# unixpickle/learn-nerf

Hardware: AMD Instinct MI355X
Metric: ray-samples/s (NeRF train step: fwd + bwd + Adam, 4096 rays x 192 samples per GPU) (higher is better)
Workload: dtype bf16; 1 GPU; vanilla NeRF coarse64+fine128 train step (BASELINE.json configs[1]); rays_per_gpu=4096, coarse_samples=64, fine_samples=128, global_batch_rays=4096, parallelism=dp1, precision=bf16 MFMA, fp32 accumulate/master weights

## Files before the change

### learn-nerf_amd/csrc/layout_host.cpp

```cpp
#include <stdint.h>
#include <string.h>

#include "dense_plan.h"
#include "fast_math.h"
#include "hashgrid_plan.h"
#include "nerf_wgrad.h"
#include "ngp_layout.h"

using namespace lnrf;

static WgradList wgrad_list_of(int which, int64_t n_tiles) {
  return which == 0 ? wgrad_list_split(n_tiles) : which == 1 ? wgrad_list_ls_finish(n_tiles)
       : which == 2 ? wgrad_list_ref_trunk(n_tiles) : which == 3 ? wgrad_list_ref_normal(n_tiles)
                                                                 : wgrad_list_ref_dir(n_tiles);
}
template <int NXF, int NYF, int WI, int WO>
static int64_t wgrad_count_owners(const WgradProblem& pb, int32_t* count, int64_t n) {
  int64_t outside = 0;
  int64_t i;
  auto hit = [&](bool owned) {
    if (!owned) return;
    if (i >= 0 && i < n) ++count[i];
    else ++outside;
  };
  for (int w = 0; w < kWaves; ++w)
    for (int j = 0; j < kWgradWaveTiles<NXF, NYF, WI, WO>; ++j) {
      const WgradTile tile = wgrad_tile<NXF, NYF, WI, WO>(w, j);
      if (!tile.real) continue;
      for (int lane = 0; lane < 64; ++lane) {
        const int colr = lane & 31, hh = lane >> 5;
        const WgradOwner<NerfWgradEpi, WgradProblem> own(pb, tile.ot, colr);
        if (tile.bias && pb.do_bias) hit(own.bias(hh, i));
        for (int qq = 0; qq < 16; ++qq) hit(own.weight(pb, tile.it, hh, qq, i));
      }
    }
  return outside;
}

template <int P>
static int64_t ngp_count_owners(const NgpWgradProblem& pb, int64_t dense_off, int32_t* count, int64_t n) {
  constexpr int NO = kNgpWgrad[P].nyf / 2, NT = ngp_wgrad_tiles(P);
  int64_t outside = 0;
  auto hit = [&](int part, int64_t i) {
    if (i >= 0 && i < n) ++count[part * n + i];
    else ++outside;
  };
  for (int w4 = 0; w4 < 4; ++w4)
    for (int lane = 0; lane < 64; ++lane) {
      const int colr = lane & 31, hh = lane >> 5;
      const int tile_id = w4 % NT, part = w4 / NT;
      const int it = tile_id / NO, ot = tile_id % NO;
      int out_idx = -1, out_dim = 1;
      int64_t w_off = 0, b_off = 0;
      NgpWgradEpi::cols(pb, ot, colr, out_idx, out_dim, w_off, b_off);
      w_off -= dense_off;
      b_off -= dense_off;
      if (it == 0 && hh == 0 && out_idx >= 0) hit(part, b_off + out_idx);
      for (int qq = 0; qq < 16; ++qq) {
        const int r = ngp_acc_row(qq, hh);
        const int f = 2 * it + (r >> 4);
        const int in_idx = NgpWgradEpi::row(pb, f, r & 15);
        if (out_idx >= 0 && in_idx >= 0) hit(part, w_off + (int64_t)in_idx * out_dim + out_idx);
      }
    }
  return outside;
}
static bool ngp_enc_dim_ok(int enc_dim) { return enc_dim >= 1 && enc_dim <= 32; }
// ... 19 lines not shown
                                                                                             : fwd_cons_base(s);
}
int lnrf_host_bwd_layer_info(int t, int what) {
  return what == 0 ? bwd_nk(t) : what == 1 ? bwd_no(t) : what == 2 ? bwd_base(t) : bwd_dense(t);
}
int lnrf_host_fwd_weight_index(int g, int lane, int j) { return fwd_stream_index(g, lane, j, false); }
int lnrf_host_bwd_weight_index(int g, int lane, int j) { return bwd_stream_index(g, lane, j, false); }
int lnrf_host_fwd_bias_index(int i) { return bias_block_index(i, false); }
int lnrf_host_nrm_frags(void) { return kNrmFrags; }
int lnrf_host_nrm_weight_index(int g, int lane, int j) { return nrm_stream_index(g, lane, j); }
int64_t lnrf_host_stream_indices(int stream, int ref, int32_t* out) {
  const int frags[8] = {kFwdFrags, kBwdFrags, kFwd3Frags, 0, kNrmFrags, kDirFwdFrags, kDirBwdFrags, 0};
  if (stream < 0 || stream > 7) return -1;
  if (stream == 3 || stream == 7) {
    const int n = stream == 3 ? kBiasFloats : kDirBiasFloats;
    for (int i = 0; out && i < n; ++i) out[i] = stream == 3 ? bias_block_index(i, ref != 0) : dir_bias_index(i);
    return n;
  }
  const int64_t n = (int64_t)frags[stream] * 512;
  for (int64_t e = 0; out && e < n; ++e) {
    const int g = (int)(e >> 9), lane = (int)((e >> 3) & 63), j = (int)(e & 7);
    out[e] = stream == 0 ? fwd_stream_index(g, lane, j, ref != 0) : stream == 1 ? bwd_stream_index(g, lane, j, ref != 0)
           : stream == 2 ? fwd3_stream_index(g, lane, j, ref != 0) : stream == 4 ? nrm_stream_index(g, lane, j)
           : stream == 5 ? dir_fwd_weight_index(g, lane, j) : dir_bwd_weight_index(g, lane, j);
  }
  return n;
}
int64_t lnrf_host_pack_offset(int what) {
  const int64_t v[17] = {kPackFwdOff, kPackBwdOff, kPackBiasOff, kPackBytes, kPack3BiasOff, kPack3Bytes,
                         kRefPackNrmOff, kRefPackDirFwdOff, kRefPackDirBwdOff, kRefPackDirBiasOff, kRefPackBytes,
                         kRef3FwdOff, kRef3BiasOff, kRef3NrmOff, kRef3DirOff, kRef3DirBiasOff, kRef3Bytes};
  return what >= 0 && what < 17 ? v[what] : -1;
}
int lnrf_host_xemb_feat(int ks, int h, int j) { return xemb_feat(ks, h, j); }
int lnrf_host_save_slot(int what, int arg) {
  return what == 0 ? kSaveXin : what == 1 ? kSaveH + 16 * arg : what == 2 ? kSaveZ : what == 3 ? kSaveDin
       : what == 4 ? kSaveH10 : what == 5 ? kSaveMask : kSaveSlots;
}
int lnrf_host_grad_slot(int what, int arg) {
  return what == 0 ? kGradDy11 : what == 1 ? kGradDy10m : what == 2 ? grad_dy_slot(arg) : kGradSlots;
}
int lnrf_host_dir_slot(int what) {
  const int v[7] = {kDirSaveXin, kDirSaveH, kDirSaveMask, kDirSaveSlots, kDirGradDy10, kDirGradDy9, kDirGradSlots};
  return what >= 0 && what < 7 ? v[what] : -1;
}
int lnrf_host_demb_feat(int ks, int h, int j) { return demb_feat(ks, h, j); }
int lnrf_host_hidden_feat(int ks, int h, int j) { return hidden_feat(ks, h, j); }
int lnrf_host_dump_info(int what) { return what == 0 ? kFragBytes : what == 1 ? kTileCols : kWaves; }
int lnrf_host_mask_bit(int ks, int j) { return 16 * (ks >> 1) + 8 * (ks & 1) + j; }
int lnrf_host_dump_lane_off(int slot, int c, int hh) { return dump_lane_off(slot, c, hh); }
void lnrf_host_sincos_pe(float r, float* s, float* c) { lnrf::sincos_pe(r, s, c); }

int lnrf_host_wgrad_const(int what) {
  const int v[8] = {kWgradMaxBlocks, kSlabMaxTiles, kSlabMaxTO, kParamCount, kDirW9, kDirB9, kDirW10, kDirB10};
  return v[what];
}
int lnrf_host_wgrad_list(int which, int64_t n_tiles, int32_t* out) {
  const WgradList list = wgrad_list_of(which, n_tiles);
  for (int i = 0; i < list.args.n_problems; ++i) {
    const WgradProblem& pb = list.args.p[i];
    int32_t* o = out + 6 * i;
    o[0] = pb.first_block; o[1] = pb.n_blocks; o[4] = pb.do_bias; o[5] = 0;
    switch (pb.shape) {
#define X(name, id, NXF, NYF, WI, WO, SPI) case name: o[2] = WgShape<name>::TI * WgShape<name>::TO; o[3] = WgShape<name>::TO; break;
      LNRF_WGRAD_SHAPES(X, X)
#undef X
      default: return -1;
    }
    switch (pb.shape) {
#define X(name) case name:
      LNRF_WGRAD_LS_SHAPES(X, X) o[5] = 1; break;
#undef X
      default: break;
    }
  }
  return list.args.n_problems;
}
int64_t lnrf_host_ngp_stream_indices(int stream, int enc_dim, int32_t* out) {
  if (stream < 0 || stream > 2 || !ngp_enc_dim_ok(enc_dim)) return -1;
  const NgpOffsets off = ngp_offsets(enc_dim, 0);
  const int ne = ngp_ne(enc_dim);
  const int64_t n = stream == 2 ? kNgpBiasFloats : (int64_t)kNgpStreamFrags * 512;
  for (int64_t e = 0; out && e < n; ++e) {
    const int g = (int)(e >> 9), lane = (int)((e >> 3) & 63), j = (int)(e & 7);
    out[e] = (int32_t)(stream == 0 ? ngp_fwd_stream_index(g, lane, j, off, enc_dim, ne)
                     : stream == 1 ? ngp_bwd_stream_index(g, lane, j, off, enc_dim, ne) : ngp_bias_index((int)e, off));
  }
  return n;
}
int64_t lnrf_host_ngp_pack_offset(int what) {
  const int64_t v[7] = {kNgpPackBiasOff, kNgpPackBytes, kNgpSplitBiasOff, kNgpSplitBytes, kNgpStreamFrags,
                        kNgpSplitMaxFrags / 2, kNgpMaxParts};
  return what >= 0 && what < 7 ? v[what] : -1;
}
int64_t lnrf_host_ngp_wgrad_owners(int enc_dim, int32_t* count, int64_t n) {
  if (!ngp_enc_dim_ok(enc_dim)) return -1;
  const int64_t dense_off = 1001;
  const NgpWgradArgs a = ngp_wgrad_args(ngp_offsets(enc_dim, dense_off), enc_dim);
  return ngp_count_owners<0>(a.p[0], dense_off, count, n) + ngp_count_owners<1>(a.p[1], dense_off, count, n) +
         ngp_count_owners<2>(a.p[2], dense_off, count, n) + ngp_count_owners<3>(a.p[3], dense_off, count, n) +
         ngp_count_owners<4>(a.p[4], dense_off, count, n);
}
int lnrf_host_ngp_parts_plan(int enc_dim, int32_t* out) {
  if (!ngp_enc_dim_ok(enc_dim)) return -1;
  const NgpPartsPlan pl = ngp_parts_plan(ngp_offsets(enc_dim, 1001), 1001);
  for (int i = 0; i < kNgpLayers; ++i) {
    int32_t* o = out + 4 * i;
// ... 86 lines not shown
```

### learn-nerf_amd/csrc/nerf_bwd_ls.hip

```cpp
#include "nerf_chain.h"

namespace lnrf {

constexpr int kLsWaves = 4;
constexpr int kLsThreads = kLsWaves * 64;
constexpr int kLsStages = 8;
constexpr int kLsLag = 2;
constexpr int kLsDist = kLsLag + 1;
constexpr int kLsBufs = kLsDist + 1;
constexpr int kLsTileBytes = 32 * kFragBytes;
constexpr int kLsPollOff = kLsBufs * kLsTileBytes;
constexpr int kLsLds = kLsPollOff + 5 * 256;
constexpr unsigned kLsMaxSpins = 1u << 18;
constexpr int kLsSlabWaveFloats = 16 * kSlabTileFloats + 2 * 64;
constexpr int64_t kLsSlabBlockBytes = (int64_t)kLsWaves * kLsSlabWaveFloats * (int64_t)sizeof(float);
constexpr int kLsCounterStride = 32;

struct LsJob {
  const char* packed;
  const char* save;
  char* gdump;
  unsigned* counters;
  float* slabs;
  unsigned* status;
// ... 350 lines not shown
  const int out = 32 * b + colr;
  if (bias) {
    bs += __shfl_xor(bs, 32, 64);
    if (hh == 0) grads[dense_b_off(l) + out] += bs;
  }
  const int it = 2 * w + a;
#pragma unroll
  for (int qq = 0; qq < 16; ++qq) {
    const int r = (qq & 3) + 8 * (qq >> 2) + 4 * hh;
    grads[dense_w_off(l) + (int64_t)(32 * it + r) * 256 + out] += acc[qq];
  }
}
__global__ __launch_bounds__(256) void nerf_ls_reduce_kernel(const float* __restrict__ slabs, int pipelines,
                                                             float* __restrict__ grads) {
  __shared__ float lds[3 * 17 * 64];
  ls_fold_block<4>(blockIdx.x, slabs, pipelines, grads, lds);
}

struct LsFoldArgs {
  WgradArgs w[2];
  const float* small_slabs[2];
  const float* ls_slabs[2];
  float* grads[2];
  int pipelines[2];
};
__global__ __launch_bounds__(64 * kSlabReduceWaves) void nerf_ls_fold_kernel(LsFoldArgs a) {
  __shared__ float lds[(kSlabReduceWaves - 1) * 17 * 64];
  const int k = blockIdx.y;
  const int n_small = a.w[k].n_problems * kWaves * kSlabMaxTiles;
  const int bid = blockIdx.x;
  if (bid < n_small) {
    const int prob = bid / (kWaves * kSlabMaxTiles), w = bid / kSlabMaxTiles % kWaves, j = bid % kSlabMaxTiles;
    const WgradProblem pb = a.w[k].p[prob];
    switch (pb.shape) {
#define X(name)                                                                                                    \
  case name:                                                                                                       \
    wgrad_reduce_tile<WgShape<name>::NXF, WgShape<name>::NYF, WgShape<name>::WI, WgShape<name>::WO, NerfWgradEpi>( \
        pb, w, j, a.small_slabs[k], a.grads[k], lds);                                                              \
    break;
      LNRF_WGRAD_LS_SHAPES(X, default: X)
#undef X
    }
  } else if (bid - n_small < kLsStages * 64) {
    ls_fold_block<kSlabReduceWaves>(bid - n_small, a.ls_slabs[k], a.pipelines[k], a.grads[k], lds);
  }
}

struct BwdHeadSeq {
  static constexpr int count = bwd_cons_base(2);
  static constexpr int at(int c) { return bwd_seq(c); }
};
constexpr int kBwdHeadStages = bwd_base(2) / kStageFrags;

__global__ __launch_bounds__(kThreads) void nerf_bwd_head_kernel(
    const char* __restrict__ packed, const char* __restrict__ save, const float* __restrict__ density,
    const float* __restrict__ rgb, const float* __restrict__ g_density, const float* __restrict__ g_rgb,
    int64_t M, int64_t n_tiles, char* __restrict__ gdump, unsigned* __restrict__ zero_words, int n_zero_words) {
  const int tid = threadIdx.x;
  const int lane = tid & 63;
  const int wave = __builtin_amdgcn_readfirstlane(tid >> 6);
  const int64_t tile = (int64_t)blockIdx.x * kWaves + wave;
  for (int i = blockIdx.x * kThreads + tid; i < n_zero_words; i += gridDim.x * kThreads) zero_words[i] = 0u;
  Ring<kBwdHeadStages, BwdHeadSeq> ring;
  ring.stream = packed + kPackBwdOff;
  ring.wave = wave;
  ring.lane = lane;
  const DumpAddr gd{gdump, n_tiles, tile, lane & 31, lane >> 5, kGradTileSlots};
  bwd_chain_tile<true>(ring, gd, save, n_tiles, density, rgb, g_density, g_rgb, M, tile, lane);
}

}

using namespace lnrf;

#ifdef LNRF_TIMELINE
extern "C" int lnrf_debug_set_ls_timeline(void* buf) {
  hipError_t e = hipMemcpyToSymbol(HIP_SYMBOL(lnrf::g_ls_timeline_buf), &buf, sizeof(buf));
  return e == hipSuccess ? LNRF_OK : hip_fail(e, "hipMemcpyToSymbol(g_ls_timeline_buf)");
}
#endif

constexpr int kLsMaxPipelines = 64;
static int ls_pipelines_for_device(int need, int* out) {
  int cus = 0;
  if (int rc = cu_count(&cus)) return rc;
  *out = cus / kLsStages < kLsMaxPipelines ? cus / kLsStages : kLsMaxPipelines;
  if (*out < need) {
    set_error("layer-stationary backward: the device has too few CUs for a pipeline of 8 per model");
    return LNRF_ERR_UNSUPPORTED;
  }
  return LNRF_OK;
}

constexpr int64_t kLsCounterWords = (int64_t)kLsMaxPipelines * kLsStages * kLsCounterStride;
constexpr int64_t kLsCounterBytes = (kLsCounterWords + 64) * (int64_t)sizeof(unsigned);
struct LsScratch {
  int64_t small_slabs, counters, status, ls_slabs, bytes;
};
static LsScratch ls_scratch(int64_t m) {
  LsScratch s;
  s.small_slabs = (int64_t)kGradSlots * padded_tiles(m) * kFragBytes;
  s.counters = s.small_slabs + kWgradSlabBytes;
  s.status = s.counters + kLsCounterWords * (int64_t)sizeof(unsigned);
  s.ls_slabs = s.counters + kLsCounterBytes;
  s.bytes = s.ls_slabs + (int64_t)kLsMaxPipelines * kLsStages * kLsSlabBlockBytes;
  return s;
}
static LsJob ls_job(const void* packed, const void* save, void* scratch, int64_t m, int pipelines) {
  const LsScratch at = ls_scratch(m);
  char* sc = (char*)scratch;
  return LsJob{(const char*)packed, (const char*)save, sc, reinterpret_cast<unsigned*>(sc + at.counters),
               reinterpret_cast<float*>(sc + at.ls_slabs), reinterpret_cast<unsigned*>(sc + at.status), padded_tiles(m),
               pipelines};
}

extern "C" int64_t lnrf_nerf_bwd_ls_scratch_bytes(const lnrf_nerf_shape* s, int64_t m) {
  return nerf_shape_fused(s) ? ls_scratch(m).bytes : -1;
}
extern "C" int64_t lnrf_nerf_bwd_ls_status_offset(const lnrf_nerf_shape* s, int64_t m) {
  return nerf_shape_fused(s) ? ls_scratch(m).status : -1;
}
int64_t lnrf::ls_scratch_bytes(int64_t m) { return ls_scratch(m).bytes; }
float* lnrf::ls_small_slabs(void* scratch, int64_t m) {
  return reinterpret_cast<float*>((char*)scratch + ls_scratch(m).small_slabs);
}

int lnrf::launch_ls_pipeline(const void* packed, const void* save, void* scratch, int64_t m, float* grads, hipStream_t st) {
  int total = 0;
  int rc = ls_pipelines_for_device(1, &total);
  if (!rc) rc = set_max_dynamic_lds(nerf_bwd_ls_kernel, kLsLds);
  if (rc) return rc;
  LsArgs a;
  a.n_jobs = 1;
  a.total_pipelines = total;
  a.job[0] = a.job[1] = ls_job(packed, save, scratch, m, total);
  hipError_t e = hipMemsetAsync(a.job[0].counters, 0, kLsCounterBytes, st);
  if (e != hipSuccess) return hip_fail(e, "hipMemsetAsync(counters)");
  hipLaunchKernelGGL(nerf_bwd_ls_kernel, dim3((unsigned)(total * kLsStages)), dim3(kLsThreads), kLsLds, st, a);
  LNRF_LAUNCH_CHECK();
  hipLaunchKernelGGL(nerf_ls_reduce_kernel, dim3(kLsStages * 64), dim3(256), 0, st, (const float*)a.job[0].slabs, total, grads);
  LNRF_LAUNCH_CHECK();
  return LNRF_OK;
}

namespace {
struct LsModel {
  const void* packed;
  const void* save;
  const float *density, *rgb, *g_density, *g_rgb;
  int64_t m;
  void* scratch;
  float* grads;
};
}

static int ls_backward(const LsModel* mdl, int n_models, int phases, hipStream_t st) {
  constexpr int kHeadLds = kRingBytes + round_up(kBiasFloats * 4, 1024);
  int total = 0;
  int rc = ls_pipelines_for_device(n_models, &total);
  if (!rc) rc = set_max_dynamic_lds(nerf_bwd_head_kernel, kHeadLds);
  if (!rc) rc = set_max_dynamic_lds(nerf_bwd_ls_kernel, kLsLds);
  if (rc) return rc;
  int pipes[2] = {total, 0};
  if (n_models == 2) {
    const double share = (double)mdl[0].m / (double)(mdl[0].m + mdl[1].m);
    pipes[0] = (int)(total * share + 0.5);
    if (pipes[0] < 1) pipes[0] = 1;
    if (pipes[0] > total - 1) pipes[0] = total - 1;
    pipes[1] = total - pipes[0];
  }
  LsArgs a;
  a.n_jobs = n_models;
  a.total_pipelines = total;
  for (int k = 0; k < n_models; ++k) {
    const LsModel& md = mdl[k];
    const LsJob& j = a.job[k] = ls_job(md.packed, md.save, md.scratch, md.m, pipes[k]);
    if (phases & 1) {
      hipLaunchKernelGGL(nerf_bwd_head_kernel, dim3((unsigned)(j.n_tiles / kWaves)), dim3(kThreads), kHeadLds, st, j.packed,
                         j.save, md.density, md.rgb, md.g_density, md.g_rgb, md.m, j.n_tiles, j.gdump, j.counters,
                         (phases & 2) ? (int)(kLsCounterBytes / sizeof(unsigned)) : 0);
      LNRF_LAUNCH_CHECK();
    }
    if ((phases & 3) == 2) {
      hipError_t e = hipMemsetAsync(j.counters, 0, kLsCounterBytes, st);
      if (e != hipSuccess) return hip_fail(e, "hipMemsetAsync(counters)");
    }
  }
  if (n_models == 1) a.job[1] = a.job[0];
  if (phases & 2) {
    hipLaunchKernelGGL(nerf_bwd_ls_kernel, dim3((unsigned)(total * kLsStages)), dim3(kLsThreads), kLsLds, st, a);
    LNRF_LAUNCH_CHECK();
  }
  if (!(phases & 4)) return LNRF_OK;
  LsFoldArgs fold;
  for (int k = 0; k < n_models; ++k) {
    const LsModel& md = mdl[k];
    const LsJob& j = a.job[k];
    const WgradList w = wgrad_list_ls_finish(j.n_tiles);
    float* small_slabs = ls_small_slabs(md.scratch, md.m);
    rc = launch_nerf_wgrad(w, md.save, md.scratch, j.n_tiles, md.grads, st, WgLayout{kSaveTileSlots, kGradTileSlots, 1},
                           small_slabs, false, false);
    if (rc) return rc;
    fold.w[k] = w.args;
    fold.small_slabs[k] = small_slabs;
    fold.ls_slabs[k] = j.slabs;
    fold.grads[k] = md.grads;
    fold.pipelines[k] = pipes[k];
  }
  if (n_models == 1) {
    fold.w[1] = fold.w[0]; fold.small_slabs[1] = fold.small_slabs[0]; fold.ls_slabs[1] = fold.ls_slabs[0];
    fold.grads[1] = fold.grads[0]; fold.pipelines[1] = fold.pipelines[0];
  }
  const int gx = fold.w[0].n_problems * kWaves * kSlabMaxTiles + kLsStages * 64;
  hipLaunchKernelGGL(nerf_ls_fold_kernel, dim3((unsigned)gx, (unsigned)n_models), dim3(64 * kSlabReduceWaves), 0, st, fold);
  LNRF_LAUNCH_CHECK();
  return LNRF_OK;
}

extern "C" int lnrf_nerf_mlp_bwd_ls(const lnrf_nerf_shape* shape, const void* packed, const void* save,
                                    const float* density, const float* rgb, const float* g_density,
                                    const float* g_rgb, int64_t m, void* scratch, float* grads, int32_t phases,
                                    lnrf_stream_t stream) {
  LNRF_REQUIRE_NERF_SHAPE(shape);
  LNRF_CHECK_ARG(packed && save && density && rgb && g_density && g_rgb && scratch && grads, "null pointer");
  LNRF_CHECK_ARG(m >= 0, "bad m");
  if (m == 0) return LNRF_OK;
  LNRF_CHECK_ARG(phases >= 1 && phases <= 7, "phases: bit 0 head, bit 1 pipeline, bit 2 small problems + fold");
  const LsModel md{packed, save, density, rgb, g_density, g_rgb, m, scratch, grads};
  return ls_backward(&md, 1, phases, as_stream(stream));
}

extern "C" int lnrf_nerf_mlp_bwd_ls2(const lnrf_nerf_shape* shape, const void* packed_a, const void* save_a,
                                     const float* density_a, const float* rgb_a, const float* g_density_a,
                                     const float* g_rgb_a, int64_t m_a, void* scratch_a, float* grads_a,
                                     const void* packed_b, const void* save_b, const float* density_b,
                                     const float* rgb_b, const float* g_density_b, const float* g_rgb_b, int64_t m_b,
                                     void* scratch_b, float* grads_b, int32_t phases, lnrf_stream_t stream) {
  LNRF_REQUIRE_NERF_SHAPE(shape);
  LNRF_CHECK_ARG(packed_a && save_a && density_a && rgb_a && g_density_a && g_rgb_a && scratch_a && grads_a, "null pointer");
  LNRF_CHECK_ARG(packed_b && save_b && density_b && rgb_b && g_density_b && g_rgb_b && scratch_b && grads_b, "null pointer");
  LNRF_CHECK_ARG(m_a > 0 && m_b > 0, "both models need evaluations (use lnrf_nerf_mlp_bwd_ls for one)");
  const LsModel md[2] = {{packed_a, save_a, density_a, rgb_a, g_density_a, g_rgb_a, m_a, scratch_a, grads_a},
                         {packed_b, save_b, density_b, rgb_b, g_density_b, g_rgb_b, m_b, scratch_b, grads_b}};
  LNRF_CHECK_ARG(phases >= 1 && phases <= 7, "phases: bit 0 head, bit 1 pipeline, bit 2 small problems + fold");
  return ls_backward(md, 2, phases, as_stream(stream));
}
```

### learn-nerf_amd/csrc/nerf_chain.h

```cpp
#pragma once
#include "fused_chain.h"

namespace lnrf {

template <class Put>
__device__ __forceinline__ void x_encode(const float (&px)[3], int h, Put put) {
  static_for<4>([&](auto ks_) {
    constexpr int ks = decltype(ks_)::value;
#pragma unroll
    for (int pp = 0; pp < 4; ++pp) {
      const int p = 4 * ks + pp;
      float s = 0.0f, co = 0.0f;
      if (p < kXPairs) {
        const int pg = kXPairs * h + p;
        const int cd = pg / kXFreqs, f = pg - kXFreqs * cd;
        const float v = cd == 0 ? px[0] : (cd == 1 ? px[1] : px[2]);
        sincos_pe(v * (float)(1 << f), &s, &co);
      }
      put(ks_, 2 * pp, s);
      put(ks_, 2 * pp + 1, co);
    }
  });
}

template <int S, bool BIAS, class RING, class Epi>
__device__ __forceinline__ void trunk_layer(RING& ring, int h, const bf16x8 (&xe)[4], const bf16x8 (&in)[16], Epi epi) {
  chain_layer<fwd_cons_base(S), fwd_nk(S), fwd_no(S)>(
      ring,
      [&](auto o_) {
        if constexpr (BIAS) return bias_acc(fwd_bias_base(S) + 32 * decltype(o_)::value, h);
        else return zero_acc();
      },
      [&](auto k_) -> bf16x8 {
        constexpr int ks = decltype(k_)::value;
        if constexpr (S == 0) return xe[ks];
        else if constexpr (ks < 16) return in[ks];
        else return xe[ks - 16];
      },
      epi);
}
template <int S, class RING, class Epi>
__device__ __forceinline__ void trunk_layer_split(RING& ring, int h, const bf16x8 (&xe_hi)[4], const bf16x8 (&xe_lo)[4],
                                                  const bf16x8 (&inh)[16], const bf16x8 (&inl)[16], Epi epi) {
  chain_layer_split<fwd_cons_base(S), fwd_nk(S), fwd_no(S)>(
      ring, [&](auto o_) { return bias_acc(fwd_bias_base(S) + 32 * decltype(o_)::value, h); },
      [&](auto k_) -> bf16x8 {
        constexpr int ks = decltype(k_)::value;
        if constexpr (S == 0) return xe_hi[ks];
        else if constexpr (ks < 16) return inh[ks];
        else return xe_hi[ks - 16];
      },
      [&](auto k_) -> bf16x8 {
        constexpr int ks = decltype(k_)::value;
        if constexpr (S == 0) return xe_lo[ks];
        else if constexpr (ks < 16) return inl[ks];
        else return xe_lo[ks - 16];
      },
      epi);
}
template <int O>
__device__ __forceinline__ void masked_out_tile(const f32x16& acc, const uint4& mk, bf16x8 (&out)[16], const DumpAddr& gd,
                                                int slot0) {
  const unsigned mb = mask_word(mk, O);
  out[2 * O] = masked_frag<0>(acc, mb, 16 * (O & 1));
  out[2 * O + 1] = masked_frag<1>(acc, mb, 16 * (O & 1));
  gd.store(slot0 + 2 * O, frag_to_bits(out[2 * O]));
  gd.store(slot0 + 2 * O + 1, frag_to_bits(out[2 * O + 1]));
}
template <int C0, int L, class RING>
__device__ __forceinline__ void hidden_back(RING& ring, bf16x8 (&in)[16], bf16x8 (&out)[16], const uint4& mk,
                                            const DumpAddr& gd) {
  chain_layer<C0, 16, 8>(
      ring, [&](auto) { return zero_acc(); }, [&](auto k_) -> bf16x8 { return in[decltype(k_)::value]; },
      [&](auto o_, const f32x16& acc) { masked_out_tile<decltype(o_)::value>(acc, mk, out, gd, grad_dy_slot(L - 1)); });
}

struct BwdSeq {
  static constexpr int count = kBwdUsed;
  static constexpr int at(int c) { return bwd_seq(c); }
};
constexpr int kBwdStages = kBwdFrags / kStageFrags;

template <bool HEAD_ONLY = false, class RING>
__device__ __forceinline__ void bwd_chain_tile(RING& ring, const DumpAddr& gd, const char* __restrict__ save,
                                               int64_t save_tiles, const float* __restrict__ density,
                                               const float* __restrict__ rgb, const float* __restrict__ g_density,
                                               const float* __restrict__ g_rgb, int64_t M, int64_t tile, int lane) {
  const int c = lane & 31, h = lane >> 5;
  const int64_t m = tile * kTileCols + c;
  const bool valid = m < M;

  float gy11[3] = {0, 0, 0}, gy9 = 0.0f;
  if (valid && h == 0) {
#pragma unroll
    for (int k = 0; k < 3; ++k) {
      const float y = rgb[m * 3 + k];
      gy11[k] = g_rgb[m * 3 + k] * (1.0f - y * y);
    }
    gy9 = g_density[m] * -expm1f(-density[m]);
  }
  uint4 relu_mask[9];
#pragma unroll
  for (int i = HEAD_ONLY ? 8 : 0; i < 9; ++i)
    relu_mask[i] = *mask_at(save, kSaveMask + i, tile, save_tiles, kSaveTileSlots, lane);
  __syncthreads();
  ring.prologue();
  LNRF_TL_STAMP(ring);

  bf16x8 a0[16], a1[16];

  bf16x8 dy11 = zero_frag();
  dy11[0] = (__bf16)gy11[0];
  dy11[1] = (__bf16)gy11[1];
  dy11[2] = (__bf16)gy11[2];
  gd.store(kGradDy11, frag_to_bits(dy11));
  gd.store(kGradDy11 + 1, frag_to_bits(zero_frag()));

  chain_layer<bwd_cons_base(0), bwd_nk(0), bwd_no(0)>(
      ring, [&](auto) { return zero_acc(); }, [&](auto) -> bf16x8 { return dy11; },
      [&](auto o_, const f32x16& acc) {
        masked_out_tile<decltype(o_)::value>(acc, relu_mask[8], a0, gd, kGradDy10m);
      });
  bf16x8 dlogit = zero_frag();
  dlogit[0] = (__bf16)gy9;
  gd.store(kGradDy10m + 8, frag_to_bits(dlogit));
  gd.store(kGradDy10m + 9, frag_to_bits(zero_frag()));

  chain_layer<bwd_cons_base(1), bwd_nk(1), bwd_no(1)>(
      ring, [&](auto) { return zero_acc(); },
      [&](auto k_) -> bf16x8 {
        constexpr int ks = decltype(k_)::value;
        if constexpr (ks < 8) return a0[ks];
        else return dlogit;
      },
      [&](auto o_, const f32x16& acc) {
        constexpr int o = decltype(o_)::value;
        a1[2 * o] = acc_to_frag<0, false>(acc);
// ... 24 lines not shown
```

### learn-nerf_amd/csrc/nerf_wgrad.h

```cpp
#pragma once
#include "nerf_layout.h"

namespace lnrf {
using namespace nl;

constexpr int kSlabMaxTiles = 9, kSlabMaxTO = 4;
constexpr int kSlabTileFloats = 64 * 16;
constexpr int kSlabWaveFloats = kSlabMaxTiles * kSlabTileFloats + kSlabMaxTO * 64;
constexpr int64_t kSlabBlockBytes = (int64_t)kWaves * kSlabWaveFloats * (int64_t)sizeof(float);
constexpr int kWgradMaxBlocks = 512;
constexpr int64_t kWgradSlabBytes = kWgradMaxBlocks * kSlabBlockBytes;

#define LNRF_WGRAD_SHAPES(X, X_ELSE)                                                                      \
  X(WG_HIDDEN, 0, 16, 16, 4, 2, 2)                                          \
  X(WG_Z_DY10M, 1, 16, 10, 4, 2, 2)                                                        \
  X(WG_XEMB, 2, 4, 16, 2, 4, 3)                                             \
  X(WG_DEMB_DY10M, 3, 2, 10, 1, 8, 5)                                                  \
  X(WG_DIR9, 5, 18, 8, 4, 2, 2)                                                     \
  X(WG_ZD_DY10M, 6, 18, 10, 4, 2, 2)                                             \
  X(WG_XEMB_DY0_DY5, 7, 4, 32, 2, 4, 2)                                          \
  X_ELSE(WG_H128_DY3, 4, 8, 2, 4, 2, 6)
#define LNRF_WGRAD_LS_SHAPES(X, X_ELSE) X(WG_XEMB_DY0_DY5) X(WG_ZD_DY10M) X_ELSE(WG_H128_DY3)

enum WgradShape : int {
#define X(name, id, nxf, nyf, wi, wo, spi) name = id,
  LNRF_WGRAD_SHAPES(X, X)
#undef X
};
template <WgradShape S>
struct WgShape;
#define X(name, id, nxf, nyf, wi, wo, spi)                                              \
  template <>                                                                           \
  struct WgShape<name> {                                                                \
    static constexpr int NXF = nxf, NYF = nyf, WI = wi, WO = wo, SPI = spi;             \
    static constexpr int TI = (nxf / 2 + wi - 1) / wi, TO = (nyf / 2 + wo - 1) / wo;  \
  };
LNRF_WGRAD_SHAPES(X, X)
#undef X

enum { ROW_HIDDEN = 0, ROW_XEMB = 1, ROW_DEMB = 2, ROW_Z_DEMB = 3 };
enum { COL_256 = 0, COL_DY10M = 1, COL_DY11 = 2, COL_EXPLICIT = 3, COL_DY0_DY5 = 4 };
struct WgradProblem {
  WgradShape shape;
  int x_slot0;
  int y_slot0;
  int dense;
  int row_map;
  int row_off;
  int col_map;
  int do_bias;
  int first_block, n_blocks;
  int w_off, b_off, out_dim, n_rows;
};
constexpr int kMaxProblems = 13;
struct WgradArgs {
  WgradProblem p[kMaxProblems];
  int n_problems;
};

struct NerfWgradEpi {
  static NL_HD void cols(const WgradProblem& pb, int ot, int colr, int& out_idx, int& out_dim, int64_t& w_off,
                         int64_t& b_off) {
    int dense_w = pb.dense;
    if (pb.col_map == COL_DY10M) {
// ... 66 lines not shown
    row_lim = EPI::row_limit(pb, ot);
  }
  NL_HD bool bias(int hh, int64_t& idx) const {
    idx = b_off + out_idx;
    return hh == 0 && out_idx >= 0 && b_off >= 0;
  }
  NL_HD bool weight(const PB& pb, int it, int hh, int qq, int64_t& idx) const {
    const int r = (qq & 3) + 8 * (qq >> 2) + 4 * hh;
    const int f = 2 * it + (r >> 4);
    const int in_idx = EPI::row(pb, f, r & 15);
    idx = w_off + (int64_t)in_idx * out_dim + out_idx;
    return out_idx >= 0 && in_idx >= 0 && in_idx < row_lim;
  }
};

struct WgradList {
  WgradArgs args;
  int blocks = 0;
  int64_t cap;
  explicit WgradList(int64_t n_tiles) : cap((n_tiles + 5) / 6) { args.n_problems = 0; }

  WgradProblem& add(int want, WgradShape shape, int xs, int ys, int dense, int row_map, int row_off, int col_map,
                    int do_bias) {
    WgradProblem& p = args.p[args.n_problems++];
    p = WgradProblem{shape, xs, ys, dense, row_map, row_off, col_map, do_bias, blocks, (int)(want < cap ? want : cap),
                     0, 0, 0, 0};
    blocks += p.n_blocks;
    return p;
  }
  void hidden(int want, int l, int do_bias) {
    add(want, WG_HIDDEN, kSaveH + (l - 1) * 16, grad_dy_slot(l), l, ROW_HIDDEN, 0, COL_256, do_bias);
  }
  void xemb_dy0_dy5(int want, int do_bias) {
    add(want, WG_XEMB_DY0_DY5, kSaveXin, grad_dy_slot(0), 0, ROW_XEMB, 0, COL_DY0_DY5, do_bias);
  }
  void zd_dy10m(int want) { add(want, WG_ZD_DY10M, kSaveZ, kGradDy10m, 10, ROW_Z_DEMB, 0, COL_DY10M, 1); }
  void h10_dy11(int want) { add(want, WG_H128_DY3, kSaveH10, kGradDy11, 11, ROW_HIDDEN, 0, COL_DY11, 1); }
  void explicit_at(int want, WgradShape shape, int xs, int ys, int out_dim, int n_rows, int w_off, int b_off) {
    WgradProblem& p = add(want, shape, xs, ys, 0, ROW_HIDDEN, 0, COL_EXPLICIT, 1);
    p.w_off = w_off; p.b_off = b_off; p.out_dim = out_dim; p.n_rows = n_rows;
  }
};

inline WgradList wgrad_list_split(int64_t n_tiles) {
  WgradList w(n_tiles);
  for (int l = 1; l <= 8; ++l) w.hidden(l <= 4 ? 48 : 47, l, 1);
  w.add(39, WG_Z_DY10M, kSaveZ, kGradDy10m, 10, ROW_HIDDEN, 0, COL_DY10M, 1);
  w.add(30, WG_XEMB, kSaveXin, grad_dy_slot(0), 0, ROW_XEMB, 0, COL_256, 1);
  w.add(30, WG_XEMB, kSaveXin, grad_dy_slot(5), 5, ROW_XEMB, 256, COL_256, 0);
  w.add(18, WG_DEMB_DY10M, kSaveDin, kGradDy10m, 10, ROW_DEMB, 256, COL_DY10M, 0);
  w.h10_dy11(15);
  return w;
}
inline WgradList wgrad_list_ls_finish(int64_t n_tiles) {
  WgradList w(n_tiles);
  w.xemb_dy0_dy5(256 * 36 / 74, 1);
  w.zd_dy10m(256 * 28 / 74);
  w.h10_dy11(256 * 10 / 74);
  return w;
}
inline WgradList wgrad_list_ref_trunk(int64_t n_tiles) {
  WgradList w(n_tiles);
  w.xemb_dy0_dy5(256, 1);
  return w;
}
inline WgradList wgrad_list_ref_normal(int64_t n_tiles) {
  WgradList w(n_tiles);
  for (int l = 1; l <= 8; ++l) w.hidden(28, l, 0);
  w.xemb_dy0_dy5(32, 0);
  return w;
}
inline WgradList wgrad_list_ref_dir(int64_t n_tiles) {
  WgradList w(n_tiles);
  w.explicit_at(200, WG_DIR9, kDirSaveXin, kDirGradDy9, kDirHidden, kDirIn, kDirW9, kDirB9);
  w.explicit_at(56, WG_H128_DY3, kDirSaveH, kDirGradDy10, 3, kDirHidden, kDirW10, kDirB10);
  return w;
}

}
```

Measured before the change: 186.5 million ray-samples/s.

## Fuse head weight-gradient GEMMs into the backward head kernel

The backward head kernel now runs as a persistent grid sized to the CU count. After each tile group's head chain it reuses the dy fragments staged in LDS plus the saved z/demb/h10 activations to accumulate the ZD_DY10M and H10_DY11 weight gradients and their bias sums in registers, using transpose LDS reads and MFMA. These partial sums are written to slabs that the fold stage reduces, and the later wgrad launch now only handles the x_emb problem. This avoids re-reading the dumped gradients and activations in a separate wgrad pass, at the cost of more LDS, extra register pressure and fewer head blocks.

Measured after the change: 187.7 million ray-samples/s, median of 6. About the same (+0.6%).

```diff
diff --git a/learn-nerf_amd/csrc/layout_host.cpp b/learn-nerf_amd/csrc/layout_host.cpp
--- a/learn-nerf_amd/csrc/layout_host.cpp
+++ b/learn-nerf_amd/csrc/layout_host.cpp
@@ -10,9 +10,11 @@
 using namespace lnrf;
 
 static WgradList wgrad_list_of(int which, int64_t n_tiles) {
-  return which == 0 ? wgrad_list_split(n_tiles) : which == 1 ? wgrad_list_ls_finish(n_tiles)
+  const int hb = ls_head_blocks(n_tiles, kLsHeadMaxBlocks);
+  return which == 0 ? wgrad_list_split(n_tiles) : which == 1 ? wgrad_list_ls_fold(n_tiles, hb)
        : which == 2 ? wgrad_list_ref_trunk(n_tiles) : which == 3 ? wgrad_list_ref_normal(n_tiles)
-                                                                 : wgrad_list_ref_dir(n_tiles);
+       : which == 4 ? wgrad_list_ref_dir(n_tiles) : which == 5 ? wgrad_list_ls_finish(n_tiles)
+       : wgrad_list_ls_head(n_tiles, hb, wgrad_list_ls_finish(n_tiles).blocks);
 }
 template <int NXF, int NYF, int WI, int WO>
 static int64_t wgrad_count_owners(const WgradProblem& pb, int32_t* count, int64_t n) {
@@ -138,7 +140,8 @@
 void lnrf_host_sincos_pe(float r, float* s, float* c) { lnrf::sincos_pe(r, s, c); }
 
 int lnrf_host_wgrad_const(int what) {
-  const int v[8] = {kWgradMaxBlocks, kSlabMaxTiles, kSlabMaxTO, kParamCount, kDirW9, kDirB9, kDirW10, kDirB10};
+  const int v[9] = {kLsFoldMaxBlocks, kSlabMaxTiles, kSlabMaxTO, kParamCount, kDirW9, kDirB9, kDirW10, kDirB10,
+                    kWgradMaxBlocks};
   return v[what];
 }
 int lnrf_host_wgrad_list(int which, int64_t n_tiles, int32_t* out) {
diff --git a/learn-nerf_amd/csrc/nerf_bwd_ls.hip b/learn-nerf_amd/csrc/nerf_bwd_ls.hip
--- a/learn-nerf_amd/csrc/nerf_bwd_ls.hip
+++ b/learn-nerf_amd/csrc/nerf_bwd_ls.hip
@@ -426,21 +426,225 @@
 };
 constexpr int kBwdHeadStages = bwd_base(2) / kStageFrags;
 
-__global__ __launch_bounds__(kThreads) void nerf_bwd_head_kernel(
+constexpr int kHwPassTiles = 2;
+constexpr int kHwPasses = kWaves / kHwPassTiles;
+constexpr int kHwXF = 26;
+static_assert(kSaveDin == kSaveZ + 16 && kSaveH10 == kSaveZ + 18 && (kSaveZ & 1) == 0, "the staged slots are neighbours");
+constexpr int kHwXFrags = kHwPassTiles * kHwXF;
+constexpr int kHwPerWave = (kHwXFrags + kWaves - 1) / kWaves;
+constexpr int kHwYOff = kHwXFrags * kFragBytes;
+constexpr int kHwYTile = 11 * kFragBytes;
+constexpr int kHwBiasOff = kHwYOff + kWaves * kHwYTile;
+constexpr int kHwLds = kHwBiasOff + 3 * kThreads * 4;
+static_assert(kHwYOff >= kRingBytes && kHwLds <= 160 * 1024, "LDS plan");
+static_assert(((kHwPassTiles - 1) * kHwXF + 9) * kFragBytes < 65536 && (kHwPassTiles - 1) * kHwYTile + 5 * kFragBytes < 65536,
+              "LDS read immediates");
+static_assert(WgShape<WG_ZD_DY10M>::TI == 3 && WgShape<WG_ZD_DY10M>::TO == 3 && WgShape<WG_ZD_DY10M>::WO == 2 &&
+                  WgShape<WG_H128_DY3>::TI == 1 && WgShape<WG_H128_DY3>::TO == 1 && WgShape<WG_H128_DY3>::WO == 2 &&
+                  kGradDy10m == 2 && kGradDy == 12,
+              "the tile-to-wave maps and slots below");
+
+struct HeadDump {
+  DumpAddr g;
+  char* ytile;
+  __device__ __forceinline__ void store(int slot, uint4 v) const {
+    if (slot == kGradDy11 + 1 || slot == kGradDy10m + 9) {
+      unsigned z = 0u;
+      asm volatile("" : "+v"(z));
+      v = make_uint4(z, z, z, z);
+    }
+    g.store(slot, v);
+    if (slot < kGradDy && slot != kGradDy11 + 1) {
+      const int pos = slot == kGradDy11 ? 10 : slot - kGradDy10m;
+      *reinterpret_cast<uint4*>(ytile + pos * kFragBytes + dump_lane_off(slot, g.c, g.hh)) = v;
+    }
+  }
+};
+
+template <int IMM>
+__device__ __forceinline__ bf16x8 tr_at(int a, int b) {
+  typedef __attribute__((address_space(3))) char lds_char;
+  typedef __attribute__((address_space(3))) s16x4 lds_s16x4;
+  lds_char* l = (lds_char*)smem;
+  const s16x4 lo = __builtin_amdgcn_ds_read_tr16_b64_v4i16((lds_s16x4*)(l + a + IMM));
+  const s16x4 hi = __builtin_amdgcn_ds_read_tr16_b64_v4i16((lds_s16x4*)(l + b + IMM));
+  typedef short s16x8 __attribute__((ext_vector_type(8)));
+  s16x8 v;
+  v[0] = lo[0]; v[1] = lo[1]; v[2] = lo[2]; v[3] = lo[3];
+  v[4] = hi[0]; v[5] = hi[1]; v[6] = hi[2]; v[7] = hi[3];
+  return __builtin_bit_cast(bf16x8, v);
+}
+struct TrBase {
+  int a, b;
+};
+
+__global__ __launch_bounds__(kThreads) void nerf_bwd_headw_kernel(
     const char* __restrict__ packed, const char* __restrict__ save, const float* __restrict__ density,
     const float* __restrict__ rgb, const float* __restrict__ g_density, const float* __restrict__ g_rgb,
-    int64_t M, int64_t n_tiles, char* __restrict__ gdump, unsigned* __restrict__ zero_words, int n_zero_words) {
+    int64_t M, int64_t n_tiles, char* __restrict__ gdump, unsigned* __restrict__ zero_words, int n_zero_words,
+    float* __restrict__ slabs, int zd_first, int h_first) {
   const int tid = threadIdx.x;
   const int lane = tid & 63;
   const int wave = __builtin_amdgcn_readfirstlane(tid >> 6);
-  const int64_t tile = (int64_t)blockIdx.x * kWaves + wave;
+  const int wi = wave >> 1, wo = wave & 1;
   for (int i = blockIdx.x * kThreads + tid; i < n_zero_words; i += gridDim.x * kThreads) zero_words[i] = 0u;
-  Ring<kBwdHeadStages, BwdHeadSeq> ring;
-  ring.stream = packed + kPackBwdOff;
-  ring.wave = wave;
-  ring.lane = lane;
-  const DumpAddr gd{gdump, n_tiles, tile, lane & 31, lane >> 5, kGradTileSlots};
-  bwd_chain_tile<true>(ring, gd, save, n_tiles, density, rgb, g_density, g_rgb, M, tile, lane);
+
+  f32x16 acc[3][3];
+#pragma unroll
+  for (int a = 0; a < 3; ++a)
+#pragma unroll
+    for (int b = 0; b < 3; ++b) acc[a][b] = zero_acc();
+  float* bias_park = reinterpret_cast<float*>(smem + kHwBiasOff) + tid;
+  bias_park[0] = bias_park[kThreads] = bias_park[2 * kThreads] = 0.0f;
+
+  auto dot2_frag = [&](float& s, const bf16x8& f) {
+    const uint4 w = frag_to_bits(f);
+    dot2_ones(s, w.x);
+    dot2_ones(s, w.y);
+    dot2_ones(s, w.z);
+    dot2_ones(s, w.w);
+  };
+
+  const int64_t n_groups = n_tiles / kWaves;
+  for (int64_t grp = blockIdx.x; grp < n_groups; grp += gridDim.x) {
+    const int64_t tile = grp * kWaves + wave;
+    {
+      Ring<kBwdHeadStages, BwdHeadSeq> ring;
+      ring.stream = packed + kPackBwdOff;
+      ring.wave = wave;
+      ring.lane = lane;
+      const HeadDump gd{DumpAddr{gdump, n_tiles, tile, lane & 31, lane >> 5, kGradTileSlots}, smem + kHwYOff + wave * kHwYTile};
+      bwd_chain_tile<true>(ring, gd, save, n_tiles, density, rgb, g_density, g_rgb, M, tile, lane);
+    }
+    __builtin_amdgcn_sched_barrier(0);
+
+    int la, lb, frag;
+    {
+      int ln = lane;
+      asm volatile("" : "+v"(ln));
+      const int g = ln >> 4, i = ln & 15, hk = g >> 1, qp = i >> 2, pc = i & 3;
+      frag = g & 1;
+      const int common = 256 * hk + 64 * (pc & 1) + 16 * qp + 8 * (pc >> 1);
+      la = common + 128 * frag;
+      lb = common + 128 * (1 - frag);
+    }
+    auto tr_base = [&](int even, int odd) {
+      TrBase t{even + odd * frag + la, even + odd * frag + lb};
+      asm("" : "+v"(t.a), "+v"(t.b));
+      return t;
+    };
+    const TrBase xw = tr_base(2 * wi * kFragBytes, kFragBytes);
+    const TrBase x8 = tr_base(16 * kFragBytes, kFragBytes);
+    const TrBase x9 = tr_base((wo ? 18 + 2 * wi : 16) * kFragBytes, kFragBytes);
+    const TrBase yw0 = tr_base(kHwYOff + 2 * wo * kFragBytes, kFragBytes);
+    const TrBase y40 = tr_base(kHwYOff + 8 * kFragBytes, kFragBytes);
+    const TrBase y90 = tr_base(kHwYOff + (wo ? 10 : 8) * kFragBytes, wo ? -kFragBytes : kFragBytes);
+
+    float bsum[3] = {bias_park[0], bias_park[kThreads], bias_park[2 * kThreads]};
+    uint4 rr[kHwPerWave];
+    auto load_x = [&](int p) {
+      const int64_t t0 = grp * kWaves + p * kHwPassTiles;
+      const __amdgpu_buffer_rsrc_t rx = __builtin_amdgcn_make_buffer_rsrc(
+          const_cast<char*>(save) + (t0 * kSaveTileSlots + kSaveZ) * (int64_t)kFragBytes, 0, 0x7FFFFFFF, 0x00020000);
+#pragma unroll
+      for (int q = 0; q < kHwPerWave; ++q) {
+        int j = wave + kWaves * q;
+        j = j < kHwXFrags ? j : kHwXFrags - 1;
+        const int u = j / kHwXF, f = j - u * kHwXF;
+        const u32x4 v = __builtin_amdgcn_raw_buffer_load_b128(rx, lane * 16, (u * kSaveTileSlots + f) * kFragBytes, 2);
+        rr[q] = make_uint4(v[0], v[1], v[2], v[3]);
+      }
+    };
+    auto write_x = [&]() {
+#pragma unroll
+      for (int q = 0; q < kHwPerWave; ++q) {
+        int j = wave + kWaves * q;
+        j = j < kHwXFrags ? j : kHwXFrags - 1;
+        *reinterpret_cast<uint4*>(&smem[j * kFragBytes + lane * 16]) = rr[q];
+      }
+    };
+    load_x(0);
+    static_for<kHwPasses>([&](auto p_) {
+      constexpr int p = decltype(p_)::value;
+      __syncthreads();
+      write_x();
+      if constexpr (p + 1 < kHwPasses) load_x(p + 1);
+      TrBase yw = yw0, y4 = y40, y9 = y90;
+      asm volatile("" : "+v"(yw.a), "+v"(yw.b), "+v"(y4.a), "+v"(y4.b), "+v"(y9.a), "+v"(y9.b));
+      yw.a += p * kHwPassTiles * kHwYTile; yw.b += p * kHwPassTiles * kHwYTile;
+      y4.a += p * kHwPassTiles * kHwYTile; y4.b += p * kHwPassTiles * kHwYTile;
+      y9.a += p * kHwPassTiles * kHwYTile; y9.b += p * kHwPassTiles * kHwYTile;
+      __syncthreads();
+      bf16x8 A[2], B[3], A9, B9;
+      A[0] = tr_at<0>(xw.a, xw.b);
+      B[0] = tr_at<0>(yw.a, yw.b);
+      B[1] = tr_at<4 * kFragBytes>(yw.a, yw.b);
+      B[2] = tr_at<0>(y4.a, y4.b);
+      A[1] = tr_at<8 * kFragBytes>(xw.a, xw.b);
+      A9 = tr_at<0>(x9.a, x9.b);
+      B9 = tr_at<0>(y9.a, y9.b);
+      __builtin_amdgcn_sched_barrier(0);
+      static_for<2 * kHwPassTiles>([&](auto n_) {
+        constexpr int n = decltype(n_)::value, P = n & 1;
+        constexpr bool more = n + 1 < 2 * kHwPassTiles;
+        constexpr int xo = (n >> 1) * kHwXF * kFragBytes + (n & 1) * 512;
+        constexpr int xn = ((n + 1) >> 1) * kHwXF * kFragBytes + ((n + 1) & 1) * 512;
+        constexpr int yn = ((n + 1) >> 1) * kHwYTile + ((n + 1) & 1) * 512;
+        static_for<3>([&](auto b_) {
+          constexpr int b = decltype(b_)::value;
+          acc[0][b] = __builtin_amdgcn_mfma_f32_32x32x16_bf16(A[P], B[b], acc[0][b], 0, 0, 0);
+          if constexpr (b < 2) dot2_frag(bsum[b], B[b]);
+          if constexpr (b == 2) A[P] = tr_at<xo>(x8.a, x8.b);
+          __builtin_amdgcn_sched_barrier(0);
+        });
+        static_for<3>([&](auto b_) {
+          constexpr int b = decltype(b_)::value;
+          acc[1][b] = __builtin_amdgcn_mfma_f32_32x32x16_bf16(A[1 - P], B[b], acc[1][b], 0, 0, 0);
+          if constexpr (b == 2 && more) {
+            A[1 - P] = tr_at<xn>(xw.a, xw.b);
+            B[2] = tr_at<yn>(y4.a, y4.b);
+          }
+          __builtin_amdgcn_sched_barrier(0);
+        });
+        static_for<2>([&](auto b_) {
+          constexpr int b = decltype(b_)::value;
+          acc[2][b] = __builtin_amdgcn_mfma_f32_32x32x16_bf16(A[P], B[b], acc[2][b], 0, 0, 0);
+          if constexpr (more) B[b] = tr_at<yn + 4 * b * kFragBytes>(yw.a, yw.b);
+          if constexpr (b == 1 && more) A[P] = tr_at<xn + 8 * kFragBytes>(xw.a, xw.b);
+          __builtin_amdgcn_sched_barrier(0);
+        });
+        acc[2][2] = __builtin_amdgcn_mfma_f32_32x32x16_bf16(A9, B9, acc[2][2], 0, 0, 0);
+        dot2_frag(bsum[2], B9);
+        if constexpr (more) {
+          A9 = tr_at<xn>(x9.a, x9.b);
+          B9 = tr_at<yn>(y9.a, y9.b);
+        }
+        __builtin_amdgcn_sched_barrier(0);
+      });
+    });
+    bias_park[0] = bsum[0];
+    bias_park[kThreads] = bsum[1];
+    bias_park[2 * kThreads] = bsum[2];
+  }
+  const float bsum[3] = {bias_park[0], bias_park[kThreads], bias_park[2 * kThreads]};
+
+  auto store_tile = [&](float* mine, int j, const f32x16& t) {
+    float4* dst = reinterpret_cast<float4*>(mine + j * kSlabTileFloats) + lane;
+#pragma unroll
+    for (int v = 0; v < 4; ++v) dst[64 * v] = make_float4(t[4 * v], t[4 * v + 1], t[4 * v + 2], t[4 * v + 3]);
+  };
+  float* __restrict__ zd = slabs + ((int64_t)(zd_first + (int)blockIdx.x) * kWaves + wave) * kSlabWaveFloats;
+  float* __restrict__ hs = slabs + ((int64_t)(h_first + (int)blockIdx.x) * kWaves + (wave - wo)) * kSlabWaveFloats;
+  static_for<8>([&](auto j_) {
+    constexpr int j = decltype(j_)::value;
+    store_tile(zd, j, acc[j / 3][j % 3]);
+  });
+  store_tile(wo ? hs : zd, wo ? 0 : 8, acc[2][2]);
+  if (wi == 0) {
+    zd[kSlabTileFloats * kSlabMaxTiles + lane] = bsum[0];
+    zd[kSlabTileFloats * kSlabMaxTiles + 64 + lane] = bsum[1];
+    (wo ? hs : zd)[kSlabTileFloats * kSlabMaxTiles + (wo ? 0 : 2 * 64) + lane] = bsum[2];
+  }
 }
 
 }
@@ -474,7 +678,7 @@
 static LsScratch ls_scratch(int64_t m) {
   LsScratch s;
   s.small_slabs = (int64_t)kGradSlots * padded_tiles(m) * kFragBytes;
-  s.counters = s.small_slabs + kWgradSlabBytes;
+  s.counters = s.small_slabs + kLsSmallSlabBytes;
   s.status = s.counters + kLsCounterWords * (int64_t)sizeof(unsigned);
   s.ls_slabs = s.counters + kLsCounterBytes;
   s.bytes = s.ls_slabs + (int64_t)kLsMaxPipelines * kLsStages * kLsSlabBlockBytes;
@@ -529,10 +733,10 @@
 }
 
 static int ls_backward(const LsModel* mdl, int n_models, int phases, hipStream_t st) {
-  constexpr int kHeadLds = kRingBytes + round_up(kBiasFloats * 4, 1024);
-  int total = 0;
+  int total = 0, cus = 0;
   int rc = ls_pipelines_for_device(n_models, &total);
-  if (!rc) rc = set_max_dynamic_lds(nerf_bwd_head_kernel, kHeadLds);
+  if (!rc) rc = cu_count(&cus);
+  if (!rc) rc = set_max_dynamic_lds(nerf_bwd_headw_kernel, kHwLds);
   if (!rc) rc = set_max_dynamic_lds(nerf_bwd_ls_kernel, kLsLds);
   if (rc) return rc;
   int pipes[2] = {total, 0};
@@ -550,9 +754,12 @@
     const LsModel& md = mdl[k];
     const LsJob& j = a.job[k] = ls_job(md.packed, md.save, md.scratch, md.m, pipes[k]);
     if (phases & 1) {
-      hipLaunchKernelGGL(nerf_bwd_head_kernel, dim3((unsigned)(j.n_tiles / kWaves)), dim3(kThreads), kHeadLds, st, j.packed,
-                         j.save, md.density, md.rgb, md.g_density, md.g_rgb, md.m, j.n_tiles, j.gdump, j.counters,
-                         (phases & 2) ? (int)(kLsCounterBytes / sizeof(unsigned)) : 0);
+      const int hb = ls_head_blocks(j.n_tiles, cus);
+      const WgradList hl = wgrad_list_ls_head(j.n_tiles, hb, wgrad_list_ls_finish(j.n_tiles).blocks);
+      hipLaunchKernelGGL(nerf_bwd_headw_kernel, dim3((unsigned)hb), dim3(kThreads), kHwLds, st, j.packed, j.save, md.density,
+                         md.rgb, md.g_density, md.g_rgb, md.m, j.n_tiles, j.gdump, j.counters,
+                         (phases & 2) ? (int)(kLsCounterBytes / sizeof(unsigned)) : 0, ls_small_slabs(md.scratch, md.m),
+                         hl.args.p[0].first_block, hl.args.p[1].first_block);
       LNRF_LAUNCH_CHECK();
     }
     if ((phases & 3) == 2) {
@@ -575,7 +782,7 @@
     rc = launch_nerf_wgrad(w, md.save, md.scratch, j.n_tiles, md.grads, st, WgLayout{kSaveTileSlots, kGradTileSlots, 1},
                            small_slabs, false, false);
     if (rc) return rc;
-    fold.w[k] = w.args;
+    fold.w[k] = wgrad_list_ls_fold(j.n_tiles, ls_head_blocks(j.n_tiles, cus)).args;
     fold.small_slabs[k] = small_slabs;
     fold.ls_slabs[k] = j.slabs;
     fold.grads[k] = md.grads;
@@ -599,7 +806,7 @@
   LNRF_CHECK_ARG(packed && save && density && rgb && g_density && g_rgb && scratch && grads, "null pointer");
   LNRF_CHECK_ARG(m >= 0, "bad m");
   if (m == 0) return LNRF_OK;
-  LNRF_CHECK_ARG(phases >= 1 && phases <= 7, "phases: bit 0 head, bit 1 pipeline, bit 2 small problems + fold");
+  LNRF_CHECK_ARG(phases >= 1 && phases <= 7, "phases: bit 0 head + its weight gradients, bit 1 pipeline, bit 2 x_emb problem + fold");
   const LsModel md{packed, save, density, rgb, g_density, g_rgb, m, scratch, grads};
   return ls_backward(&md, 1, phases, as_stream(stream));
 }
@@ -616,6 +823,6 @@
   LNRF_CHECK_ARG(m_a > 0 && m_b > 0, "both models need evaluations (use lnrf_nerf_mlp_bwd_ls for one)");
   const LsModel md[2] = {{packed_a, save_a, density_a, rgb_a, g_density_a, g_rgb_a, m_a, scratch_a, grads_a},
                          {packed_b, save_b, density_b, rgb_b, g_density_b, g_rgb_b, m_b, scratch_b, grads_b}};
-  LNRF_CHECK_ARG(phases >= 1 && phases <= 7, "phases: bit 0 head, bit 1 pipeline, bit 2 small problems + fold");
+  LNRF_CHECK_ARG(phases >= 1 && phases <= 7, "phases: bit 0 head + its weight gradients, bit 1 pipeline, bit 2 x_emb problem + fold");
   return ls_backward(md, 2, phases, as_stream(stream));
 }
diff --git a/learn-nerf_amd/csrc/nerf_chain.h b/learn-nerf_amd/csrc/nerf_chain.h
--- a/learn-nerf_amd/csrc/nerf_chain.h
+++ b/learn-nerf_amd/csrc/nerf_chain.h
@@ -58,8 +58,8 @@
       },
       epi);
 }
-template <int O>
-__device__ __forceinline__ void masked_out_tile(const f32x16& acc, const uint4& mk, bf16x8 (&out)[16], const DumpAddr& gd,
+template <int O, class GD>
+__device__ __forceinline__ void masked_out_tile(const f32x16& acc, const uint4& mk, bf16x8 (&out)[16], const GD& gd,
                                                 int slot0) {
   const unsigned mb = mask_word(mk, O);
   out[2 * O] = masked_frag<0>(acc, mb, 16 * (O & 1));
@@ -67,9 +67,9 @@
   gd.store(slot0 + 2 * O, frag_to_bits(out[2 * O]));
   gd.store(slot0 + 2 * O + 1, frag_to_bits(out[2 * O + 1]));
 }
-template <int C0, int L, class RING>
+template <int C0, int L, class RING, class GD>
 __device__ __forceinline__ void hidden_back(RING& ring, bf16x8 (&in)[16], bf16x8 (&out)[16], const uint4& mk,
-                                            const DumpAddr& gd) {
+                                            const GD& gd) {
   chain_layer<C0, 16, 8>(
       ring, [&](auto) { return zero_acc(); }, [&](auto k_) -> bf16x8 { return in[decltype(k_)::value]; },
       [&](auto o_, const f32x16& acc) { masked_out_tile<decltype(o_)::value>(acc, mk, out, gd, grad_dy_slot(L - 1)); });
@@ -81,8 +81,8 @@
 };
 constexpr int kBwdStages = kBwdFrags / kStageFrags;
 
-template <bool HEAD_ONLY = false, class RING>
-__device__ __forceinline__ void bwd_chain_tile(RING& ring, const DumpAddr& gd, const char* __restrict__ save,
+template <bool HEAD_ONLY = false, class RING, class GD>
+__device__ __forceinline__ void bwd_chain_tile(RING& ring, const GD& gd, const char* __restrict__ save,
                                                int64_t save_tiles, const float* __restrict__ density,
                                                const float* __restrict__ rgb, const float* __restrict__ g_density,
                                                const float* __restrict__ g_rgb, int64_t M, int64_t tile, int lane) {
diff --git a/learn-nerf_amd/csrc/nerf_wgrad.h b/learn-nerf_amd/csrc/nerf_wgrad.h
--- a/learn-nerf_amd/csrc/nerf_wgrad.h
+++ b/learn-nerf_amd/csrc/nerf_wgrad.h
@@ -10,6 +10,8 @@
 constexpr int64_t kSlabBlockBytes = (int64_t)kWaves * kSlabWaveFloats * (int64_t)sizeof(float);
 constexpr int kWgradMaxBlocks = 512;
 constexpr int64_t kWgradSlabBytes = kWgradMaxBlocks * kSlabBlockBytes;
+constexpr int kLsFoldMaxBlocks = 768;
+constexpr int64_t kLsSmallSlabBytes = kLsFoldMaxBlocks * kSlabBlockBytes;
 
 #define LNRF_WGRAD_SHAPES(X, X_ELSE)                                                                      \
   X(WG_HIDDEN, 0, 16, 16, 4, 2, 2)                                          \
@@ -182,11 +184,29 @@
   w.h10_dy11(15);
   return w;
 }
+constexpr int kLsHeadMaxBlocks = 256;
+inline int ls_head_blocks(int64_t n_tiles, int cus) {
+  int64_t g = cus < kLsHeadMaxBlocks ? cus : kLsHeadMaxBlocks;
+  if (g > n_tiles / kWaves) g = n_tiles / kWaves;
+  return (int)(g < 1 ? 1 : g);
+}
 inline WgradList wgrad_list_ls_finish(int64_t n_tiles) {
   WgradList w(n_tiles);
-  w.xemb_dy0_dy5(256 * 36 / 74, 1);
-  w.zd_dy10m(256 * 28 / 74);
-  w.h10_dy11(256 * 10 / 74);
+  w.xemb_dy0_dy5(256, 1);
+  return w;
+}
+inline WgradList wgrad_list_ls_head(int64_t n_tiles, int head_blocks, int first_block) {
+  WgradList w(n_tiles);
+  w.blocks = first_block;
+  w.zd_dy10m(head_blocks);
+  w.h10_dy11(head_blocks);
+  return w;
+}
+inline WgradList wgrad_list_ls_fold(int64_t n_tiles, int head_blocks) {
+  WgradList w = wgrad_list_ls_finish(n_tiles);
+  const WgradList h = wgrad_list_ls_head(n_tiles, head_blocks, w.blocks);
+  for (int i = 0; i < h.args.n_problems; ++i) w.args.p[w.args.n_problems++] = h.args.p[i];
+  w.blocks = h.blocks;
   return w;
 }
 inline WgradList wgrad_list_ref_trunk(int64_t n_tiles) {
```
